# pierrepaleo/sift_pyocl

Measured on AMD Instinct MI355X. Metric: SiftPlan.keypoints throughput, 4096x4096 fp32 (Mpix/s; keypoints/s in keypoints_per_s), higher is better.
Workload: dtype f32

## Files before the change

sift_pyocl_amd/csrc/k_keypoint.hpp:

```cpp
#pragma once
#include <hip/hip_runtime.h>
#include <stdint.h>
#include "k_extrema.hpp"
#include "siftmath.hpp"

namespace siftk {

struct KpRecord { float x, y, scale, angle; uint8_t desc[128]; };
static_assert(sizeof(KpRecord) == 144, "record layout");

struct GradTaps { float xa, xb, ya, yb; bool bx, by; };

__device__ __forceinline__ GradTaps gradient_fetch(const float *__restrict__ I, int x, int y, int W, int H) {
    const size_t pos = (size_t)y * W + x;
    GradTaps t;
    t.bx = (x == 0) || (x == W - 1);
    t.by = (y == 0) || (y == H - 1);
    t.xa = I[x == W - 1 ? pos : pos + 1];
    t.xb = I[x == 0 ? pos : pos - 1];
    t.ya = I[y == 0 ? pos : pos - W];
    t.yb = I[y == H - 1 ? pos : pos + W];
    return t;
}

__device__ __forceinline__ void gradient_eval(const GradTaps &t, float &mag, float &ori) {
    float gx = t.xa - t.xb, gy = t.ya - t.yb;
// ... 8 lines not shown
    gradient_eval(gradient_fetch(I, x, y, W, H), mag, ori);
}

__device__ __forceinline__ int div_exact(int idx, int d, float inv, int &rem) {
    int q = (int)((float)idx * inv);
    rem = idx - q * d;
    if (rem < 0) { q--; rem += d; }
    else if (rem >= d) { q++; rem -= d; }
    return q;
}

#define SIFT_MAX_OCTAVES 24
#define SIFT_GROUPS 3
struct Counters {
    int n_rec;
    int tail_timeout;
    unsigned rec_word[SIFT_GROUPS];
    int g_kp[SIFT_GROUPS];
    int g_out[SIFT_GROUPS];
    int desc_next[SIFT_GROUPS];
    int n_cand[SIFT_MAX_OCTAVES + 1];
    int c_scale[SIFT_MAX_OCTAVES][3];
    int o_scale[SIFT_MAX_OCTAVES][3];
    uint32_t mm[2];
    int tail_ready[8];
};

struct OctaveTable {
    const float *base;
    long long off[SIFT_MAX_OCTAVES];
    int W[SIFT_MAX_OCTAVES], H[SIFT_MAX_OCTAVES];
    const float *gmap, *omap;
};
__device__ __forceinline__ size_t map_offset(const OctaveTable &tab, int oct, int scale) {
    return (size_t)(tab.off[oct] / 2) + (size_t)(scale - 1) * tab.W[oct] * tab.H[oct];
}

struct alignas(16) RecordSink {
    KpRecord *dev, *host;
    int dev_limit, host_limit;
};

__device__ __forceinline__ void descriptor_open(Counters *cnt, int group, int n, KpRecord *records, int rec_capacity, KpRecord *host_records,
                                                int host_capacity, RecordSink *S) {
    if (threadIdx.x == 0) {
        int base = 0;
        if (cnt) {
// ... 118 lines not shown
    if (threadIdx.x < 3 * SIFT_MAX_OCTAVES) s_hist[threadIdx.x] = 0;
    __syncthreads();
    PH_MARK(0);
    const int wave = (blockIdx.x * blockDim.x + threadIdx.x) >> 6;
    const int nwaves = (nblocks * blockDim.x) >> 6;
    const float4 *pool4 = reinterpret_cast<const float4 *>(L.pool);
    __shared__ int s_pending[4], s_base;
    int pending = 0;
    auto store_pending = [&](int slot, int count) {
        __builtin_amdgcn_wave_barrier();
        for (int e = lane; e < count; e += 64)
            if (slot + e < out_capacity) { okp[slot + e] = L.obuf[e]; oaux[slot + e] = L.oaux[e]; }
        __builtin_amdgcn_wave_barrier();
    };
    auto flush_wave = [&]() {
        int slot = 0;
        if (lane == 0) slot = atomicAdd(&cnt->g_out[group], pending);
        store_pending(__shfl(slot, 0), pending);
        pending = 0;
    };
    const bool team = count < team_below;
    const int w4 = threadIdx.x >> 6;
    const int boff = team ? 64 * w4 : 0, bstep = team ? 256 : 64;
    for (int i = first + (team ? (int)blockIdx.x : wave); i < n; i += (team ? nblocks : nwaves)) {
        const float4 k = kp[i];
        const int aux = __builtin_amdgcn_readfirstlane(kp_aux[i]);
        const int scale = aux & 0xff, oct = aux >> 8;
        const int W = tab.W[oct], H = tab.H[oct], octsize = 1 << oct;
        if (!(k.y >= 0.0f)) continue;
        const float *I = tab.base + tab.off[oct] + (size_t)scale * W * H;
        const float *Gm = MAPS ? tab.gmap + map_offset(tab, oct, scale) : nullptr;
        const float *Om = MAPS ? tab.omap + map_offset(tab, oct, scale) : nullptr;
        auto taps_at = [&](int x, int y) {
            if (!MAPS) return gradient_fetch(I, x, y, W, H);
            GradTaps t = {};
            const size_t pos = (size_t)y * W + x;
            t.xa = Gm[pos]; t.xb = Om[pos];
            return t;
        };
        const int row = (int)((double)k.y + 0.5), col = (int)((double)k.z + 0.5);
        const float sigma = ori_sigma * k.w;
        const int radius = (int)((double)sigma * 3.0);
        const int rmin = max(0, row - radius), cmin = max(0, col - radius);
        const int rmax = min(row + radius, H - 2), cmax = min(col + radius, W - 2);
        const float lim = (float)(radius * radius) + 0.5f;
        const float two_s2 = 2.0f * sigma * sigma;
        const float r_two_s2 = 1.0f / two_s2;
        const bool fast_div = two_s2 >= 1e-3f && two_s2 <= 1e6f;
        const int wc = cmax - cmin + 1, hr = rmax - rmin + 1;
// ... 439 lines not shown
```

sift_pyocl_amd/csrc/k_pyramid.hpp:

```cpp
#pragma once
#include <hip/hip_runtime.h>
#include <type_traits>
#include <stdint.h>
#include "k_xcd.hpp"

namespace siftk {

__device__ __forceinline__ uint32_t f2ord(float f) {
    uint32_t u = __float_as_uint(f);
    return (u & 0x80000000u) ? ~u : (u | 0x80000000u);
}
__device__ __forceinline__ float ord2f(uint32_t u) {
    return __uint_as_float((u & 0x80000000u) ? (u & 0x7fffffffu) : ~u);
}

__global__ void minmax_init(uint32_t *mm) { mm[0] = 0xffffffffu; mm[1] = 0u; }

__device__ __forceinline__ void minmax_reset_next(uint32_t *reset, int reset_words, int reset_ones) {
    if (reset && blockIdx.x == 0)
        for (int i = threadIdx.x; i < reset_words; i += blockDim.x) reset[i] = (i == reset_ones) ? 0xffffffffu : 0u;
}

__global__ __launch_bounds__(1024) void minmax_kernel(const float *__restrict__ img, int64_t n, uint32_t *mm, uint32_t *reset = nullptr,
                                                      int reset_words = 0, int reset_ones = -1) {
    minmax_reset_next(reset, reset_words, reset_ones);
    float lo = __builtin_inff(), hi = -__builtin_inff();
    const int64_t stride = (int64_t)gridDim.x * blockDim.x;
    int64_t i = (int64_t)blockIdx.x * blockDim.x + threadIdx.x;
    const int64_t n4 = n >> 2;
    const float4 *img4 = reinterpret_cast<const float4 *>(img);
    int64_t k = i;
    for (; k + 3 * stride < n4; k += 4 * stride) {
        const float4 v0 = img4[k], v1 = img4[k + stride], v2 = img4[k + 2 * stride], v3 = img4[k + 3 * stride];
        lo = fminf(lo, fminf(fminf(fminf(v0.x, v0.y), fminf(v0.z, v0.w)), fminf(fminf(v1.x, v1.y), fminf(v1.z, v1.w))));
        lo = fminf(lo, fminf(fminf(fminf(v2.x, v2.y), fminf(v2.z, v2.w)), fminf(fminf(v3.x, v3.y), fminf(v3.z, v3.w))));
        hi = fmaxf(hi, fmaxf(fmaxf(fmaxf(v0.x, v0.y), fmaxf(v0.z, v0.w)), fmaxf(fmaxf(v1.x, v1.y), fmaxf(v1.z, v1.w))));
        hi = fmaxf(hi, fmaxf(fmaxf(fmaxf(v2.x, v2.y), fmaxf(v2.z, v2.w)), fmaxf(fmaxf(v3.x, v3.y), fmaxf(v3.z, v3.w))));
    }
    for (; k < n4; k += stride) {
        float4 v = img4[k];
        lo = fminf(fminf(lo, v.x), fminf(v.y, fminf(v.z, v.w)));
        hi = fmaxf(fmaxf(hi, v.x), fmaxf(v.y, fmaxf(v.z, v.w)));
    }
    for (int64_t k2 = (n4 << 2) + i; k2 < n; k2 += stride) {
        float v = img[k2];
        lo = fminf(lo, v);
        hi = fmaxf(hi, v);
    }
#pragma unroll
    for (int off = 32; off > 0; off >>= 1) {
        lo = fminf(lo, __shfl_xor(lo, off));
        hi = fmaxf(hi, __shfl_xor(hi, off));
    }
    __shared__ float slo[16], shi[16];
    const int wave = threadIdx.x >> 6, nwaves = (int)blockDim.x >> 6;
    if ((threadIdx.x & 63) == 0) { slo[wave] = lo; shi[wave] = hi; }
    __syncthreads();
    if (threadIdx.x == 0) {
        lo = slo[0]; hi = shi[0];
        for (int w = 1; w < nwaves; w++) { lo = fminf(lo, slo[w]); hi = fmaxf(hi, shi[w]); }
        if (lo <= hi) {
            atomicMin(&mm[0], f2ord(lo));
            atomicMax(&mm[1], f2ord(hi));
        }
    }
}

template <int DT> __device__ __forceinline__ float load_px(const void *__restrict__ base, size_t i) {
    if constexpr (DT == 0) return static_cast<const float *>(base)[i];
    else if constexpr (DT == 1) return (float)static_cast<const uint8_t *>(base)[i];
    else if constexpr (DT == 2) return (float)static_cast<const uint16_t *>(base)[i];
    else if constexpr (DT == 3) return (float)static_cast<const uint32_t *>(base)[i];
    else if constexpr (DT == 4) return (float)static_cast<const uint64_t *>(base)[i];
    else if constexpr (DT == 5) return (float)static_cast<const int32_t *>(base)[i];
    else if constexpr (DT == 6) return (float)static_cast<const int64_t *>(base)[i];
    else {
        static_assert(DT == 8, "unsupported pixel type");
        const uint8_t *q = static_cast<const uint8_t *>(base) + 3 * i;
        const float r = (float)q[0], g = (float)q[1], b = (float)q[2];
        return (0.299f * r + 0.587f * g) + 0.114f * b;
    }
}

template <int DT> struct TypedChunk {
    static constexpr int R = (DT == 8) ? 3 : ((DT == 4 || DT == 6) ? 2 : 1);
    static constexpr int PX = (DT == 1 || DT == 8) ? 16 : (DT == 2 ? 8 : 4);
};
// ... 49 lines not shown
    for (; k < nchunks; k += stride) {
        uint4 w[C::R];
#pragma unroll
        for (int r = 0; r < C::R; r++) w[r] = img4[k * C::R + r];
        typed_chunk_minmax<DT>(w, lo, hi);
    }
    for (int64_t k2 = nchunks * C::PX + i; k2 < n; k2 += stride) {
        const float v = load_px<DT>(img, (size_t)k2);
        lo = fminf(lo, v);
        hi = fmaxf(hi, v);
    }
#pragma unroll
    for (int off = 32; off > 0; off >>= 1) {
        lo = fminf(lo, __shfl_xor(lo, off));
        hi = fmaxf(hi, __shfl_xor(hi, off));
    }
    __shared__ float slo[4], shi[4];
    const int wave = threadIdx.x >> 6;
    if ((threadIdx.x & 63) == 0) { slo[wave] = lo; shi[wave] = hi; }
    __syncthreads();
    if (threadIdx.x == 0) {
        lo = fminf(fminf(slo[0], slo[1]), fminf(slo[2], slo[3]));
        hi = fmaxf(fmaxf(shi[0], shi[1]), fmaxf(shi[2], shi[3]));
        if (lo <= hi) {
            atomicMin(&mm[0], f2ord(lo));
            atomicMax(&mm[1], f2ord(hi));
        }
    }
}

template <typename T>
__global__ void convert_kernel(const T *__restrict__ in, float *__restrict__ out, int64_t n) {
    const int64_t stride = (int64_t)gridDim.x * blockDim.x;
    for (int64_t i = (int64_t)blockIdx.x * blockDim.x + threadIdx.x; i < n; i += stride) out[i] = (float)in[i];
}
__global__ void convert_rgb_kernel(const uint8_t *__restrict__ in, float *__restrict__ out, int64_t n) {
    const int64_t stride = (int64_t)gridDim.x * blockDim.x;
    for (int64_t i = (int64_t)blockIdx.x * blockDim.x + threadIdx.x; i < n; i += stride) {
        const float r = (float)in[3 * i], g = (float)in[3 * i + 1], b = (float)in[3 * i + 2];
        out[i] = (0.299f * r + 0.587f * g) + 0.114f * b;
    }
}

template <int N> struct TapsArg { float t[N]; };

template <int N, int TX_ = 128, int TY_ = 64> struct BlurGeom {
    static constexpr int TX = TX_, TY = TY_;
    static constexpr int C = (N & 1) ? N / 2 : N / 2 - 1;
    static constexpr int ROWS = TY + N - 1;
    static constexpr int COLS = TX + N - 1;
// ... 1 lines not shown
    static constexpr int NW = (N + 3 + 3) & ~3;
    static constexpr int LDS_BYTES = ROWS * PITCH * 4;
};

__device__ __forceinline__ int reflect_index(int i, int n) {
    if (i < 0) i = -i - 1;
    else if (i > n - 1) i = 2 * n - 1 - i;
    return min(max(i, 0), n - 1);
}

template <int N, bool NORM, int DT = 0, int TX = 128, int TY = 64, int VR = 8>
__global__ __launch_bounds__(256) void blur_hv_kernel(const void *__restrict__ in, float *__restrict__ out,
                                                      int W, int H, TapsArg<N> taps,
                                                      const uint32_t *__restrict__ mm,
                                                      float *__restrict__ half) {
    using G = BlurGeom<N, TX, TY>;
    static_assert(TX % 4 == 0 && 64 % (TX / 4) == 0, "the H tasks of one row must sit in one wave");
    static_assert(TY % VR == 0, "vertical tasks tile the rows");
    extern __shared__ float4 smem4[];
    float *s = reinterpret_cast<float *>(smem4);
    const int tid = threadIdx.x;
    const int x0 = blockIdx.x * G::TX, y0 = blockIdx.y * G::TY;

    float mn = 0.f, range = 1.f;
    if (NORM) { mn = ord2f(mm[0]); range = ord2f(mm[1]) - mn; }

    for (int idx = tid; idx < G::ROWS * G::COLS; idx += 256) {
        const int row = idx / G::COLS, col = idx - row * G::COLS;
        const int gy = reflect_index(y0 - G::C + row, H);
        const int gx = reflect_index(x0 - G::C + col, W);
        float v = load_px<DT>(in, (size_t)gy * W + gx);
        if (NORM) v = 255.0f * (v - mn) / range;
        s[row * G::PITCH + col] = v;
    }
    __syncthreads();

    constexpr int HT = TX / 4;
    for (int task = tid; task < G::ROWS * HT; task += 256) {
        const int row = task / HT, t = task - row * HT;
        float *rowp = s + row * G::PITCH + 4 * t;
        float w[G::NW];
#pragma unroll
        for (int k = 0; k < G::NW / 4; k++) {
            const float4 v = *reinterpret_cast<const float4 *>(rowp + 4 * k);
            w[4 * k] = v.x; w[4 * k + 1] = v.y; w[4 * k + 2] = v.z; w[4 * k + 3] = v.w;
        }
        float a0 = 0.f, a1 = 0.f, a2 = 0.f, a3 = 0.f;
#pragma unroll
        for (int q = 0; q < N; q++) {
            const float tp = taps.t[N - 1 - q];
            a0 = a0 + w[q] * tp;
            a1 = a1 + w[q + 1] * tp;
            a2 = a2 + w[q + 2] * tp;
            a3 = a3 + w[q + 3] * tp;
        }
// ... 74 lines not shown
__global__ __launch_bounds__(64 * HW + 128) void blur_team_kernel(const void *__restrict__ in, float *__restrict__ out,
                                                          int W, int H, int nblocks, int last_subs, int rows_out,
                                                          TapsArg<N> taps, const uint32_t *__restrict__ mm,
                                                          float *__restrict__ next0,
                                                          int xcd_map, int prio) {
    constexpr int NT = 128;
    using G = March2Geom<N, NT, S>;
    using SS = SubSplit<N, S>;
    static_assert(N & 1, "marching blur needs an odd tap count");
    constexpr int BUF = G::NPS * G::PITCH * 2;
    extern __shared__ float4 smem4[];
    float *sbase = reinterpret_cast<float *>(smem4);
    const int role = __builtin_amdgcn_readfirstlane((int)threadIdx.x) >= 64 * HW ? 1 : 0;
    const int tid = role ? (int)threadIdx.x - 64 * HW : (int)threadIdx.x;
    int bx = (int)blockIdx.x, by = (int)blockIdx.y;
    if (xcd_map) {
        const int gx = (int)gridDim.x;
        const int M = xcd_contiguous(bx + gx * by, gx * (int)gridDim.y);
        by = M / gx; bx = M - by * gx;
    }
    const int x0 = bx * G::TX;
    const int ys = by * rows_out;
    const int yend = min(ys + rows_out, H);
    float mn = 0.f, range = 1.f;
    if (NORM) { mn = ord2f(mm[0]); range = ord2f(mm[1]) - mn; }

    const int gx_a = reflect_index(x0 - G::C + tid, W);
    const int gx_b = reflect_index(x0 - G::C + NT + tid, W);
    int hb_rp[G::NB], hb_col[G::NB], hb_gx[G::NB];
#pragma unroll
    for (int u = 0; u < G::NB; u++) {
        const int e = tid + NT * u;
        hb_rp[u] = (e < G::NPS * G::HALO) ? e / G::HALO : 1 << 20;
        hb_col[u] = G::TX + e % G::HALO;
        hb_gx[u] = reflect_index(x0 - G::C + hb_col[u], W);
    }
    auto ld = [&](unsigned byte_off) {
        if constexpr (DT == 0) return *reinterpret_cast<const float *>(reinterpret_cast<const char *>(in) + byte_off);
        else return load_px<DT>(in, (size_t)(byte_off >> 2));
    };
    const unsigned W4 = (unsigned)W * 4u;
    auto norm2 = [&](f32x2 v) {
        if (NORM) { v.x = 255.0f * (v.x - mn) / range; v.y = 255.0f * (v.y - mn) / range; }
        return v;
    };
    f32x2 acc[N];
#pragma unroll
    for (int k = 0; k < N; k++) acc[k] = (f32x2){0.f, 0.f};
    const int gxo = x0 + 2 * tid;
    const bool vec_store = ((W & 1) == 0) && (gxo + 1 < W);
    f32x2 pa[G::NPS], pb[G::NPS], ph[G::NB];

    auto prefetch = [&](int blk, int sub, int np) {
        const int v0 = ys - G::C + blk * N + sub * SS::RB;
        if (BLUR_ABL & 4) {
#pragma unroll
            for (int rp = 0; rp < G::NPS; rp++) { pa[rp] = (f32x2){1.f, 2.f}; pb[rp] = (f32x2){3.f, 4.f}; }
#pragma unroll
            for (int u = 0; u < G::NB; u++) ph[u] = (f32x2){5.f, 6.f};
            return;
        }
        if (v0 >= 0 && v0 + 2 * np <= H) {
            unsigned oa = ((unsigned)v0 * (unsigned)W + (unsigned)gx_a) * 4u;
            unsigned ob = ((unsigned)v0 * (unsigned)W + (unsigned)gx_b) * 4u;
#pragma unroll
            for (int rp = 0; rp < G::NPS; rp++)
                if (rp < np) {
                    pa[rp].x = ld(oa); pa[rp].y = ld(oa + W4);
                    pb[rp].x = ld(ob); pb[rp].y = ld(ob + W4);
                    oa += 2u * W4; ob += 2u * W4;
                }
        } else {
#pragma unroll
            for (int rp = 0; rp < G::NPS; rp++)
                if (rp < np) {
                    const unsigned r0 = (unsigned)reflect_index(v0 + 2 * rp, H) * W4, r1 = (unsigned)reflect_index(v0 + 2 * rp + 1, H) * W4;
                    pa[rp].x = ld(r0 + 4u * gx_a); pa[rp].y = ld(r1 + 4u * gx_a);
                    pb[rp].x = ld(r0 + 4u * gx_b); pb[rp].y = ld(r1 + 4u * gx_b);
                }
        }
#pragma unroll
        for (int u = 0; u < G::NB; u++) {
            ph[u] = (f32x2){0.f, 0.f};
            if (hb_rp[u] < np) {
                ph[u].x = ld((unsigned)reflect_index(v0 + 2 * hb_rp[u], H) * W4 + 4u * hb_gx[u]);
                ph[u].y = ld((unsigned)reflect_index(v0 + 2 * hb_rp[u] + 1, H) * W4 + 4u * hb_gx[u]);
            }
        }
    };
    auto stage = [&](float *s, int np) {
#pragma unroll
        for (int rp = 0; rp < G::NPS; rp++)
            if (rp < np) {
                *reinterpret_cast<f32x2 *>(s + (rp * G::PITCH + tid) * 2) = norm2(pa[rp]);
                *reinterpret_cast<f32x2 *>(s + (rp * G::PITCH + NT + tid) * 2) = norm2(pb[rp]);
            }
#pragma unroll
        for (int u = 0; u < G::NB; u++)
            if (hb_rp[u] < np) *reinterpret_cast<f32x2 *>(s + (hb_rp[u] * G::PITCH + hb_col[u]) * 2) = norm2(ph[u]);
    };
    auto hpass = [&](float *s, int np) {
        for (int task = tid; task < ((BLUR_ABL & 1) ? 0 : np * (NT / 2)); task += 64 * HW) {
            const int rp = task / (NT / 2), t4 = task % (NT / 2);
            float *rowp = s + (rp * G::PITCH + 4 * t4) * 2;
            f32x2 w[G::NW];
            constexpr int PRE = 4;
#pragma unroll
            for (int k = 0; k < PRE && k < G::NW / 2; k++) {
                const f32x4 v = *reinterpret_cast<const f32x4 *>(rowp + 4 * k);
                w[2 * k] = v.xy; w[2 * k + 1] = v.zw;
            }
            f32x2 a0 = {0.f, 0.f}, a1 = {0.f, 0.f}, a2 = {0.f, 0.f}, a3 = {0.f, 0.f};
#pragma unroll
            for (int q = 0; q < N; q++) {
                if ((q & 1) == 0) {
                    const int k = q / 2 + PRE;
                    if (k < G::NW / 2) {
                        const f32x4 v = *reinterpret_cast<const f32x4 *>(rowp + 4 * k);
                        w[2 * k] = v.xy; w[2 * k + 1] = v.zw;
                    }
                    __builtin_amdgcn_sched_barrier(0);
                }
// ... 137 lines not shown
template <int N, int TX, int TY> struct Tile2Geom {
    static constexpr int C = N / 2;
    static constexpr int L = 8, VR = 8;
    static constexpr int ROWS = TY + N - 1, RP = ROWS / 2;
    static constexpr int COLS = TX + N - 1;
    static constexpr int PITCH = (COLS + 1) & ~1;
    static constexpr int LDS_BYTES = RP * PITCH * 8;
};

template <int N, bool NORM, int DT = 0, int TX = 32, int TY = 64>
__global__ __launch_bounds__(256) void blur_tile2_kernel(const void *__restrict__ in, float *__restrict__ out,
                                                         int W, int H, TapsArg<N> taps,
                                                         const uint32_t *__restrict__ mm,
                                                         float *__restrict__ half) {
    using G = Tile2Geom<N, TX, TY>;
    static_assert(N & 1, "odd tap counts only");
    static_assert(TY % G::VR == 0 && TX % G::L == 0 && 64 % (TX / G::L) == 0 && G::COLS <= 128, "tile shape");
    extern __shared__ float4 smem4[];
    float *s = reinterpret_cast<float *>(smem4);
    const int tid = threadIdx.x, lane = tid & 63;
    const int wave = __builtin_amdgcn_readfirstlane(tid >> 6);
    const int x0 = blockIdx.x * TX, y0 = blockIdx.y * TY;

    float mn = 0.f, range = 1.f;
    if (NORM) { mn = ord2f(mm[0]); range = ord2f(mm[1]) - mn; }

    {
        const int c1 = lane + 64;
        const bool has0 = lane < G::COLS, has1 = c1 < G::COLS;
        const int gxa = reflect_index(x0 - G::C + lane, W), gxb = reflect_index(x0 - G::C + (has1 ? c1 : lane), W);
        const int ytop = y0 - G::C;
        const bool inside = ytop >= 0 && ytop + G::ROWS <= H;
        auto fetch = [&](int gy, int gx) {
            float v = load_px<DT>(in, (size_t)gy * W + gx);
            if (NORM) v = 255.0f * (v - mn) / range;
            return v;
        };
        f32x2 *s2 = reinterpret_cast<f32x2 *>(s);
        if (inside) {
#pragma unroll 2
            for (int rp = wave; rp < G::RP; rp += 4) {
                const int gy = ytop + 2 * rp;
                if (has0) s2[rp * G::PITCH + lane] = (f32x2){fetch(gy, gxa), fetch(gy + 1, gxa)};
                if (has1) s2[rp * G::PITCH + c1] = (f32x2){fetch(gy, gxb), fetch(gy + 1, gxb)};
            }
        } else {
#pragma unroll 2
            for (int rp = wave; rp < G::RP; rp += 4) {
                const int gy0 = reflect_index(ytop + 2 * rp, H), gy1 = reflect_index(ytop + 2 * rp + 1, H);
                if (has0) s2[rp * G::PITCH + lane] = (f32x2){fetch(gy0, gxa), fetch(gy1, gxa)};
                if (has1) s2[rp * G::PITCH + c1] = (f32x2){fetch(gy0, gxb), fetch(gy1, gxb)};
            }
        }
    }
    __syncthreads();

    constexpr int HT = TX / G::L;
    for (int task = tid; task < G::RP * HT; task += 256) {
// ... 26 lines not shown
            const int gy = y0 + r0 + j;
            if (gy < H) {
                float *o = out + (size_t)gy * W + gx;
                if (vec) *reinterpret_cast<f32x2 *>(o) = acc[j];
                else {
                    if (gx < W) o[0] = acc[j].x;
                    if (gx + 1 < W) o[1] = acc[j].y;
                }
                if (half && !(gy & 1) && (gy >> 1) < (H >> 1) && (gx >> 1) < (W >> 1))
                    half[(size_t)(gy >> 1) * (W >> 1) + (gx >> 1)] = acc[j].x;
            }
        }
    }
}


__global__ void blur_generic_pass(const float *__restrict__ in, float *__restrict__ out, int W, int H,
                                  const float *__restrict__ taps, int n, int vertical,
                                  const uint32_t *__restrict__ mm, int norm) {
    const int x = blockIdx.x * blockDim.x + threadIdx.x, y = blockIdx.y;
    if (x >= W || y >= H) return;
    const int c = (n & 1) ? n / 2 : n / 2 - 1;
    float mn = 0.f, range = 1.f;
    if (norm) { mn = ord2f(mm[0]); range = ord2f(mm[1]) - mn; }
    float acc = 0.f;
    for (int j = 0; j < n; j++) {
        float v;
        if (vertical) v = in[(size_t)reflect_index(y - c + j, H) * W + x];
        else v = in[(size_t)y * W + reflect_index(x - c + j, W)];
        if (norm) v = 255.0f * (v - mn) / range;
        acc = acc + v * taps[n - 1 - j];
    }
    out[(size_t)y * W + x] = acc;
}

__global__ __launch_bounds__(256) void shrink_kernel(const float *__restrict__ in, float *__restrict__ out, int LW, int SW, int SH) {
    const int x = (blockIdx.x * 64 + (threadIdx.x & 63)) * 4;
    const int y0 = (blockIdx.y * 4 + (threadIdx.x >> 6)) * 2;
    if (x >= SW) return;
    const bool vec_in = (LW & 1) == 0 && x + 3 < SW;
    const bool vec_out = (SW & 3) == 0;
#pragma unroll
    for (int r = 0; r < 2; r++) {
        const int y = y0 + r;
        if (y >= SH) break;
        const float *src = in + (size_t)(2 * y) * LW + 2 * x;
        float *dst = out + (size_t)y * SW + x;
        if (vec_in) {
            const float4 a = *reinterpret_cast<const float4 *>(src), b = *reinterpret_cast<const float4 *>(src + 4);
            if (vec_out) *reinterpret_cast<float4 *>(dst) = make_float4(a.x, a.z, b.x, b.z);
            else { dst[0] = a.x; dst[1] = a.z; dst[2] = b.x; dst[3] = b.z; }
        } else {
            for (int k = 0; k < 4 && x + k < SW; k++) dst[k] = src[2 * k];
        }
    }
}
inline dim3 shrink_grid(int SW, int SH) { return dim3((unsigned)((SW + 255) / 256), (unsigned)((SH + 7) / 8)); }

template <int DT = 0>
__global__ void normalize_kernel(const void *__restrict__ in, float *__restrict__ out, int64_t n,
                                 const uint32_t *__restrict__ mm) {
    const float mn = ord2f(mm[0]), range = ord2f(mm[1]) - mn;
    const int64_t stride = (int64_t)gridDim.x * blockDim.x;
    for (int64_t i = (int64_t)blockIdx.x * blockDim.x + threadIdx.x; i < n; i += stride)
        out[i] = 255.0f * (load_px<DT>(in, (size_t)i) - mn) / range;
}

}
```

sift_pyocl_amd/csrc/siftmi.hip:

```cpp
#include <hip/hip_runtime.h>
#include <hip/hip_ext.h>

#include <cmath>
#include <cstdlib>
#include <cstring>
#include <algorithm>
#include <chrono>
#include <mutex>
#include <new>
#include <string>
#include <vector>

#include "host_common.hpp"
#include "k_extrema.hpp"
#include "k_keypoint.hpp"
#include "k_descriptor.hpp"
#include "k_align.hpp"
#include "k_pyramid.hpp"
#include "k_tail.hpp"
#include "siftmath.hpp"

using namespace siftk;

static_assert(sizeof(siftmi_keypoint) == 144, "siftmi_keypoint must be 144 bytes");
// ... 356 lines not shown
    }

struct Scope {
    siftmi_plan *p; size_t idx = (size_t)-1; hipStream_t st;
    bool stop_bound = false;
    Scope(siftmi_plan *pl, const char *label, bool is_blur = false, double pixels = 0, hipStream_t s = nullptr, int octave = -1, bool record_start = true) : p(pl) {
        st = s ? s : p->stream;
        if (!p->profile || (p->profile == 1 && !(is_blur && octave == 0))) return;
        if (p->n_events == p->events.size()) {
            Event e;
            hipEventCreate(&e.a); hipEventCreate(&e.b);
            p->events.push_back(e);
        }
        idx = p->n_events++;
        Event &e = p->events[idx];
        e.label = label; e.is_blur = is_blur; e.pixels = pixels; e.octave = octave; e.launches = 1;
        if (record_start) hipEventRecord(e.a, st);
    }
    ~Scope() { if (idx != (size_t)-1 && !stop_bound) hipEventRecord(p->events[idx].b, st); }
};

double tnow() { return std::chrono::duration<double, std::micro>(std::chrono::steady_clock::now().time_since_epoch()).count(); }
float minmax_decode(uint32_t u) { uint32_t v = (u & 0x80000000u) ? (u & 0x7fffffffu) : ~u; float f; memcpy(&f, &v, 4); return f; }

int grid_for(int64_t n, int block, int max_blocks) {
    int64_t g = (n + block - 1) / block;
    if (g < 1) g = 1;
    if (g > max_blocks) g = max_blocks;
    return (int)g;
}

double contrast_threshold(const siftmi_params &par) { return 0.8 * (double)par.peak_thresh; }
float octave_edge_thresh(const siftmi_params &par, int octsize) { return (octsize <= 1) ? par.edge_thresh0 : par.edge_thresh; }


struct DetectGeom { int rows = 0, blocks = 0; };
DetectGeom detect_geometry(int W, int H, int border, int rows_opt, int min_strips, int y_lo, int y_hi) {
    DetectGeom g;
    if (!(W > 2 * border && H > 2 * border)) return g;
    g.rows = rows_opt > 0 ? rows_opt : (min_strips > 0 ? extrema_strip_rows(W, H, border, min_strips) : extrema_strip_rows(W, H, border));
    const int nx = (W - 2 * border + 61) / 62, ny = ((y_lo >= 0 ? y_hi - y_lo : H - 2 * border) + g.rows - 1) / g.rows;
    g.blocks = (nx * ny + 3) / 4;
    return g;
}

void launch_extrema(hipStream_t st, bool refine, const DetectGeom &geo, const BlurPlanes &bp, int W, int H, int border, double contrast, float edth,
// ... 351 lines not shown
    if (!rc && (prio ? hipStreamCreateWithPriority(&p->stream3, hipStreamNonBlocking, prio_hi) : hipStreamCreateWithFlags(&p->stream3, hipStreamNonBlocking)) != hipSuccess) rc = fail(SIFTMI_EDEVICE, "hipStreamCreate failed");
    if (!rc && hipEventCreateWithFlags(&p->ev_p3, SIFT_SYNC_EVENT) != hipSuccess) rc = fail(SIFTMI_EDEVICE, "hipEventCreate failed");
    p->overlap = true;
    for (int o = 0; o < p->n_oct && !rc; o++) {
        hipEvent_t e;
        if (hipEventCreateWithFlags(&e, SIFT_SYNC_EVENT) != hipSuccess) rc = fail(SIFTMI_EDEVICE, "hipEventCreate failed");
        else p->ev_pyr.push_back(e);
    }
    if (!rc) rc = p->alloc(&p->tmp, N * sizeof(float));
    if (!rc && p->n_oct > 1) rc = p->alloc(&p->tmp_later, (size_t)p->ow[1] * p->oh[1] * sizeof(float));
    if (!rc && p->n_oct > 2) rc = p->alloc(&p->tmp_below, (size_t)p->ow[2] * p->oh[2] * sizeof(float));
    if (!rc) rc = p->alloc(&p->raw, N * (dtype_size(in_dtype) > 4 ? dtype_size(in_dtype) : 4));
    if (!rc && in_dtype != SIFTMI_F32) rc = p->alloc(&p->conv, N * sizeof(float));

    if (!rc) rc = p->alloc(&p->cnt_pair, 2 * sizeof(Counters));
    if (!rc) { p->cnt = p->cnt_pair; p->mm = p->cnt->mm; }
    p->tail_cand_cap = 3 * SIFT_TAIL_MAX_PIXELS;
    if (!rc) rc = p->alloc(&p->tail_cand, (size_t)SIFT_TAIL_MAX_OCT * p->tail_cand_cap * sizeof(float4));
    if (!rc) rc = grow_lists(p, nullptr);
    if (!rc) rc = compute_schedule(p);
    if (!rc) {
        Counters zero;
        memset(&zero, 0, sizeof zero);
        zero.mm[0] = 0xffffffffu;
        if (hipMemcpy(p->cnt_pair, &zero, sizeof zero, hipMemcpyHostToDevice) != hipSuccess ||
            hipMemcpy(p->cnt_pair + 1, &zero, sizeof zero, hipMemcpyHostToDevice) != hipSuccess) rc = fail(SIFTMI_EDEVICE, "counter initialisation failed");
    }
    if (!rc) { hipEventCreate(&p->ev_first); for (hipEvent_t &e : p->ev_last) hipEventCreate(&e); }
    if (rc) { std::string keep = g_err; siftmi_plan_destroy(p); g_err = keep; return rc; }
    *out = p;
    return SIFTMI_OK;
}

int siftmi_plan_destroy(siftmi_plan *p) {
    if (!p) return SIFTMI_OK;
    hipSetDevice(p->device);
    if (p->stream) hipStreamSynchronize(p->stream);
    if (p->stream2) { hipStreamSynchronize(p->stream2); hipStreamDestroy(p->stream2); }
    if (p->stream3) { hipStreamSynchronize(p->stream3); hipStreamDestroy(p->stream3); }
    if (p->ev_p3) hipEventDestroy(p->ev_p3);
    if (p->ev_det2) hipEventDestroy(p->ev_det2);
    if (p->ev_early) hipEventDestroy(p->ev_early);
    if (p->ev_maps0) hipEventDestroy(p->ev_maps0);
    for (hipEvent_t e : p->ev_pyr) hipEventDestroy(e);
    for (void *q : p->allocs) hipFree(q);
    for (GroupLists &G : p->grp)
        for (void *q : {(void *)G.kp, (void *)G.kp_aux, (void *)G.okp, (void *)G.oaux, (void *)G.cand}) if (q) hipFree(q);
// ... 365 lines not shown
        if (!w) continue;
        if (spin) {
            hipError_t q;
            while ((q = hipStreamQuery(w)) == hipErrorNotReady) __builtin_ia32_pause();
            if (q != hipSuccess) HIPCHK(q);
        }
        HIPCHK(hipStreamSynchronize(w));
    }
    HIPCHK(hipStreamSynchronize(p->stream));
    p->in_flight = false;
    HIPCHK(hipGetLastError());
    const Counters *hcp = nullptr;
    bool tail_timed_out = false;
    for (int k = 0; k < 3; k++) {
        if (!p->wait_s[k]) continue;
        const Counters &c = p->hb->c[k];
        tail_timed_out = tail_timed_out || c.tail_timeout;
        bool complete = true;
        for (int g = 0; g < SIFT_GROUPS; g++) if (((p->groups_cur >> g) & 1u) && !(c.rec_word[g] & 0x80000000u)) complete = false;
        if (complete && (!hcp || c.n_rec >= hcp->n_rec)) hcp = &c;
    }
    if (!hcp) { drain_streams(p); return fail(SIFTMI_EDEVICE, "no complete copy of the image's counters came back"); }
    const Counters &hc = *hcp;
    p->last_min = minmax_decode(hc.mm[0]); p->last_max = minmax_decode(hc.mm[1]);
    if (!tail_timed_out && p->opt.tail_fault > 0 && p->opt.tail) { p->opt.tail_fault--; tail_timed_out = true; }
    if (tail_timed_out) {
        p->opt.tail = 0;
        p->tail_timeouts++;
        drain_streams(p);
        return fail(SIFTMI_ETAILRETRY, "octave_tail_kernel timed out waiting for the previous octave; tail launches disabled for this plan");
    }
    {
        bool grown = false;
        int rc = grow_lists(p, &hc, &grown);
        if (rc) return rc;
        if (grown) return fail(SIFTMI_EGROW, "a keypoint list was grown; the image runs again");
    }
    int64_t n = 0;
    for (int g = 0; g < SIFT_GROUPS; g++) if ((p->groups_cur >> g) & 1u) n += std::min<int64_t>(hc.g_out[g], p->grp[g].cap_out);
    n = std::min<int64_t>(std::min<int64_t>(n, hc.n_rec), p->cap_rec);
    int ovf = reference_overflow(p, hc) ? 1 : 0;
    for (int g = 0; g < SIFT_GROUPS; g++)
        if (((p->groups_cur >> g) & 1u) && (hc.g_kp[g] > p->grp[g].cap_kp || hc.g_out[g] > p->grp[g].cap_out)) ovf = 1;
    if (hc.n_rec > p->cap_rec) ovf = 1;
    for (int g = 0; g < SIFT_GROUPS; g++) {
        if (!((p->groups_cur >> g) & 1u) || p->grp[g].cap_cand <= 0) continue;
        for (int o = 0; o < p->n_oct; o++)
// ... 572 lines not shown
    Options opt = g_default_options;
    opt.xcd_map = (xcd_map & 1) ? 1 : 0;
    opt.march_prio = (xcd_map & 2) ? 0 : 2;
    opt.march_wgs = march_wgs > 0 ? march_wgs : 0;
    if ((xcd_map >> 2) & 3) opt.small_blur = ((xcd_map >> 2) & 3) - 1;
    return opt;
}

}

extern "C" {

int siftmi_stage_gaussian_taps(float sigma, int32_t size, float *out) {
    if (!out) return fail(SIFTMI_EINVAL, "null argument");
    return gaussian_taps(sigma, size, out);
}

int32_t siftmi_stage_xcd_order(int32_t id, int32_t n) { return (n > 0 && id >= 0 && id < n) ? siftk::xcd_contiguous(id, n) : -1; }

int siftmi_stage_minmax_normalize(int32_t dev, const float *in, float *out, int32_t W, int32_t H, float *mn, float *mx) {
    int rc = stage_begin(dev); if (rc) return rc;
    const size_t N = (size_t)W * H;
    DevBuf a, b, mm;
    if ((rc = a.upload(in, N * 4)) || (rc = b.alloc(N * 4)) || (rc = mm.alloc(8))) return rc;
    hipLaunchKernelGGL(minmax_init, dim3(1), dim3(1), 0, 0, mm.as<uint32_t>());
    launch_minmax(nullptr, 0, SIFTMI_F32, a.p, (int64_t)N, 256, 2048, mm.as<uint32_t>(), nullptr, 0, -1);
    launch_normalize(0, SIFTMI_F32, a.p, b.as<float>(), (int64_t)N, mm.as<uint32_t>());
    if ((rc = stage_end())) return rc;
    uint32_t h[2];
    HIPCHK(hipMemcpy(h, mm.p, 8, hipMemcpyDeviceToHost));
    if (mn) *mn = minmax_decode(h[0]);
    if (mx) *mx = minmax_decode(h[1]);
    if (out) HIPCHK(hipMemcpy(out, b.p, N * 4, hipMemcpyDeviceToHost));
    return SIFTMI_OK;
}

int siftmi_stage_blur(int32_t dev, const float *in, float *out, int32_t W, int32_t H, const float *taps, int32_t ntaps) {
    int rc = stage_begin(dev); if (rc) return rc;
    if (ntaps < 1 || ntaps > 64) return fail(SIFTMI_EINVAL, "ntaps must be in 1..64");
    const size_t N = (size_t)W * H;
    DevBuf a, b, t, dt;
    if ((rc = a.upload(in, N * 4)) || (rc = b.alloc(N * 4)) || (rc = t.alloc(N * 4))) return rc;
    Taps tp;
    if ((rc = stage_taps(taps, ntaps, dt, tp))) return rc;
    if (!launch_blur_tiled<false>(g_default_options, 0, a.as<float>(), b.as<float>(), W, H, tp, nullptr))
        launch_blur_generic(0, a.as<float>(), b.as<float>(), t.as<float>(), W, H, tp, nullptr, false);
    if ((rc = stage_end())) return rc;
    HIPCHK(hipMemcpy(out, b.p, N * 4, hipMemcpyDeviceToHost));
    return SIFTMI_OK;
}

int siftmi_stage_blur_ex(int32_t dev, const void *in, int32_t in_dtype, float *out, int32_t W, int32_t H, const float *taps, int32_t ntaps,
                         int32_t norm, int32_t xcd_map, int32_t march_wgs, int32_t *kernel_used) {
    int rc = stage_begin(dev); if (rc) return rc;
    if (!in || !out || !taps || W < 1 || H < 1) return fail(SIFTMI_EINVAL, "null argument or empty plane");
    if (ntaps < 1 || ntaps > 64) return fail(SIFTMI_EINVAL, "ntaps must be in 1..64");
    const size_t esz = dtype_size(in_dtype);
    if (!esz || in_dtype == SIFTMI_F64) return fail(SIFTMI_EINVAL, "input format %d has no fused blur", in_dtype);
    if (in_dtype != SIFTMI_F32 && !(norm && ntaps == 15)) return fail(SIFTMI_EINVAL, "typed frames enter through the normalising 15-tap blur only");
    const size_t N = (size_t)W * H;
    DevBuf a, b, t, dt, mm;
    if ((rc = a.upload(in, N * esz)) || (rc = b.alloc(N * 4)) || (rc = t.alloc(N * 4)) || (rc = mm.alloc(8))) return rc;
    Taps tp;
    if ((rc = stage_taps(taps, ntaps, dt, tp))) return rc;
    const Options opt = stage_blur_options(xcd_map, march_wgs);
    uint32_t *mmp = mm.as<uint32_t>();
    if (norm) {
        hipLaunchKernelGGL(minmax_init, dim3(1), dim3(1), 0, 0, mmp);
        launch_minmax(nullptr, 0, in_dtype, a.p, (int64_t)N, 256, in_dtype == SIFTMI_F32 ? 2048 : 256, mmp, nullptr, 0, -1);
    }
    BlurForm used = BLUR_NONE;
    if (in_dtype != SIFTMI_F32) {
        SIFTMI_TYPED_DISPATCH(in_dtype, used = launch_init_blur_dt<DT>(opt, 0, (const void *)a.p, b.as<float>(), W, H, tp, mmp));
        if (used == BLUR_NONE) return fail(SIFTMI_EINVAL, "no fused blur for input format %d", in_dtype);
    } else {
        used = norm ? launch_blur_tiled<true>(opt, 0, a.as<float>(), b.as<float>(), W, H, tp, mmp)
                    : launch_blur_tiled<false>(opt, 0, a.as<float>(), b.as<float>(), W, H, tp, mmp);
        if (used == BLUR_NONE) launch_blur_generic(0, a.as<float>(), b.as<float>(), t.as<float>(), W, H, tp, mmp, norm != 0);
    }
    if ((rc = stage_end())) return rc;
    if (kernel_used) *kernel_used = used;
    HIPCHK(hipMemcpy(out, b.p, N * 4, hipMemcpyDeviceToHost));
    return SIFTMI_OK;
}

int siftmi_stage_blur_handoff(int32_t dev, const float *in, float *out, float *half, int32_t W, int32_t H, const float *taps, int32_t ntaps,
                              int32_t xcd_map, int32_t march_wgs, int32_t *kernel_used) {
    int rc = stage_begin(dev); if (rc) return rc;
    if (!in || !out || !half || !taps || W < 1 || H < 1) return fail(SIFTMI_EINVAL, "null argument or empty plane");
    if (ntaps < 1 || ntaps > 64) return fail(SIFTMI_EINVAL, "ntaps must be in 1..64");
    const size_t N = (size_t)W * H;
// ... 305 lines not shown
```

Measured before the change: 22070.

## Spread min/max atomics over strided slots, divide by reciprocal, prefetch keypoints

The global min/max reduction now publishes into 32 slots spaced apart in memory instead of two words, which reduces atomic contention from many blocks. Consumers fold the slots back with a wave shuffle or a serial loop, and the host folds them as well. Normalisation replaces the per-pixel division with a reciprocal-based divide that falls back to true division when the operands are out of range. Separately, the descriptor loop prefetches the next keypoint record one iteration ahead. The cost is a larger counter struct and an extra fold at every consumer.

```diff
diff --git a/sift_pyocl_amd/csrc/k_keypoint.hpp b/sift_pyocl_amd/csrc/k_keypoint.hpp
--- a/sift_pyocl_amd/csrc/k_keypoint.hpp
+++ b/sift_pyocl_amd/csrc/k_keypoint.hpp
@@ -2,6 +2,7 @@
 #include <hip/hip_runtime.h>
 #include <stdint.h>
 #include "k_extrema.hpp"
+#include "k_pyramid.hpp"
 #include "siftmath.hpp"
 
 namespace siftk {
@@ -56,7 +57,7 @@
     int n_cand[SIFT_MAX_OCTAVES + 1];
     int c_scale[SIFT_MAX_OCTAVES][3];
     int o_scale[SIFT_MAX_OCTAVES][3];
-    uint32_t mm[2];
+    alignas(128) uint32_t mm[MM_WORDS];
     int tail_ready[8];
 };
 
@@ -221,9 +222,15 @@
     const bool team = count < team_below;
     const int w4 = threadIdx.x >> 6;
     const int boff = team ? 64 * w4 : 0, bstep = team ? 256 : 64;
-    for (int i = first + (team ? (int)blockIdx.x : wave); i < n; i += (team ? nblocks : nwaves)) {
-        const float4 k = kp[i];
-        const int aux = __builtin_amdgcn_readfirstlane(kp_aux[i]);
+    const int istep = team ? nblocks : nwaves;
+    int i = first + (team ? (int)blockIdx.x : wave);
+    float4 k_next = make_float4(0.f, 0.f, 0.f, 0.f);
+    int aux_next = 0;
+    if (i < n) { k_next = kp[i]; aux_next = kp_aux[i]; }
+    for (; i < n; i += istep) {
+        const float4 k = k_next;
+        const int aux = __builtin_amdgcn_readfirstlane(aux_next);
+        if (i + istep < n) { k_next = kp[i + istep]; aux_next = kp_aux[i + istep]; }
         const int scale = aux & 0xff, oct = aux >> 8;
         const int W = tab.W[oct], H = tab.H[oct], octsize = 1 << oct;
         if (!(k.y >= 0.0f)) continue;
diff --git a/sift_pyocl_amd/csrc/k_pyramid.hpp b/sift_pyocl_amd/csrc/k_pyramid.hpp
--- a/sift_pyocl_amd/csrc/k_pyramid.hpp
+++ b/sift_pyocl_amd/csrc/k_pyramid.hpp
@@ -3,6 +3,7 @@
 #include <type_traits>
 #include <stdint.h>
 #include "k_xcd.hpp"
+#include "siftmath.hpp"
 
 namespace siftk {
 
@@ -14,11 +15,62 @@
     return __uint_as_float((u & 0x80000000u) ? (u & 0x7fffffffu) : ~u);
 }
 
-__global__ void minmax_init(uint32_t *mm) { mm[0] = 0xffffffffu; mm[1] = 0u; }
+#define MM_SLOTS 32
+#define MM_STRIDE 32
+#define MM_WORDS (MM_SLOTS * MM_STRIDE)
+__global__ void minmax_init(uint32_t *mm) {
+    for (int i = threadIdx.x; i < MM_WORDS; i += blockDim.x) mm[i] = (i % MM_STRIDE == 0) ? 0xffffffffu : 0u;
+}
+__device__ __forceinline__ void minmax_publish(uint32_t *mm, float lo, float hi) {
+    if (lo <= hi) {
+        uint32_t *slot = mm + (blockIdx.x % MM_SLOTS) * MM_STRIDE;
+        atomicMin(&slot[0], f2ord(lo));
+        atomicMax(&slot[1], f2ord(hi));
+    }
+}
+__device__ __forceinline__ uint2 minmax_fold_wave(const uint32_t *__restrict__ mm) {
+    static_assert(MM_SLOTS == 32, "the fold reads one slot per lane of half a wave");
+    const uint2 w = *reinterpret_cast<const uint2 *>(mm + (threadIdx.x & (MM_SLOTS - 1)) * MM_STRIDE);
+    uint32_t lo = w.x, hi = w.y;
+#pragma unroll
+    for (int off = MM_SLOTS / 2; off > 0; off >>= 1) {
+        lo = min(lo, (uint32_t)__shfl_xor((int)lo, off));
+        hi = max(hi, (uint32_t)__shfl_xor((int)hi, off));
+    }
+    return make_uint2((uint32_t)__builtin_amdgcn_readfirstlane((int)lo), (uint32_t)__builtin_amdgcn_readfirstlane((int)hi));
+}
+__device__ __forceinline__ uint2 minmax_fold_thread(const uint32_t *__restrict__ mm) {
+    uint32_t lo = 0xffffffffu, hi = 0u;
+    for (int s = 0; s < MM_SLOTS; s++) { lo = min(lo, mm[s * MM_STRIDE]); hi = max(hi, mm[s * MM_STRIDE + 1]); }
+    return make_uint2(lo, hi);
+}
+
+#define NORM_NUM_MIN_BITS 0x26800000u
+struct NormScale { float mn, range, rb; bool fast; };
+__device__ __forceinline__ NormScale norm_scale_of(uint2 folded) {
+    NormScale n;
+    n.mn = ord2f(folded.x); n.range = ord2f(folded.y) - n.mn;
+    n.fast = n.range >= 0x1p-126f && n.range <= 0x1p64f;
+    n.rb = 1.0f / n.range;
+    return n;
+}
+__device__ __forceinline__ float norm_num(const NormScale &n, float v) { return 255.0f * (v - n.mn); }
+__device__ __forceinline__ bool norm_num_slow(float a) {
+    const uint32_t u = __float_as_uint(a);
+    return u - 1u < NORM_NUM_MIN_BITS - 1u || (u >> 31);
+}
+__device__ __forceinline__ float norm_value(const NormScale &n, float v) {
+    const float a = norm_num(n, v);
+    if (n.fast && !norm_num_slow(a)) return siftmath::div_by_reciprocal(a, n.range, n.rb);
+    return a / n.range;
+}
 
 __device__ __forceinline__ void minmax_reset_next(uint32_t *reset, int reset_words, int reset_ones) {
     if (reset && blockIdx.x == 0)
-        for (int i = threadIdx.x; i < reset_words; i += blockDim.x) reset[i] = (i == reset_ones) ? 0xffffffffu : 0u;
+        for (int i = threadIdx.x; i < reset_words; i += blockDim.x) {
+            const unsigned m = (unsigned)(i - reset_ones);
+            reset[i] = (reset_ones >= 0 && m < MM_WORDS && m % MM_STRIDE == 0) ? 0xffffffffu : 0u;
+        }
 }
 
 __global__ __launch_bounds__(1024) void minmax_kernel(const float *__restrict__ img, int64_t n, uint32_t *mm, uint32_t *reset = nullptr,
@@ -59,10 +111,7 @@
     if (threadIdx.x == 0) {
         lo = slo[0]; hi = shi[0];
         for (int w = 1; w < nwaves; w++) { lo = fminf(lo, slo[w]); hi = fmaxf(hi, shi[w]); }
-        if (lo <= hi) {
-            atomicMin(&mm[0], f2ord(lo));
-            atomicMax(&mm[1], f2ord(hi));
-        }
+        minmax_publish(mm, lo, hi);
     }
 }
 
@@ -158,10 +207,7 @@
     if (threadIdx.x == 0) {
         lo = fminf(fminf(slo[0], slo[1]), fminf(slo[2], slo[3]));
         hi = fmaxf(fmaxf(shi[0], shi[1]), fmaxf(shi[2], shi[3]));
-        if (lo <= hi) {
-            atomicMin(&mm[0], f2ord(lo));
-            atomicMax(&mm[1], f2ord(hi));
-        }
+        minmax_publish(mm, lo, hi);
     }
 }
 
@@ -209,15 +255,15 @@
     const int tid = threadIdx.x;
     const int x0 = blockIdx.x * G::TX, y0 = blockIdx.y * G::TY;
 
-    float mn = 0.f, range = 1.f;
-    if (NORM) { mn = ord2f(mm[0]); range = ord2f(mm[1]) - mn; }
+    NormScale ns = {};
+    if (NORM) ns = norm_scale_of(minmax_fold_wave(mm));
 
     for (int idx = tid; idx < G::ROWS * G::COLS; idx += 256) {
         const int row = idx / G::COLS, col = idx - row * G::COLS;
         const int gy = reflect_index(y0 - G::C + row, H);
         const int gx = reflect_index(x0 - G::C + col, W);
         float v = load_px<DT>(in, (size_t)gy * W + gx);
-        if (NORM) v = 255.0f * (v - mn) / range;
+        if (NORM) v = norm_value(ns, v);
         s[row * G::PITCH + col] = v;
     }
     __syncthreads();
@@ -338,8 +384,8 @@
     const int x0 = bx * G::TX;
     const int ys = by * rows_out;
     const int yend = min(ys + rows_out, H);
-    float mn = 0.f, range = 1.f;
-    if (NORM) { mn = ord2f(mm[0]); range = ord2f(mm[1]) - mn; }
+    NormScale ns = {};
+    if (NORM) ns = norm_scale_of(minmax_fold_wave(mm));
 
     const int gx_a = reflect_index(x0 - G::C + tid, W);
     const int gx_b = reflect_index(x0 - G::C + NT + tid, W);
@@ -356,10 +402,6 @@
         else return load_px<DT>(in, (size_t)(byte_off >> 2));
     };
     const unsigned W4 = (unsigned)W * 4u;
-    auto norm2 = [&](f32x2 v) {
-        if (NORM) { v.x = 255.0f * (v.x - mn) / range; v.y = 255.0f * (v.y - mn) / range; }
-        return v;
-    };
     f32x2 acc[N];
 #pragma unroll
     for (int k = 0; k < N; k++) acc[k] = (f32x2){0.f, 0.f};
@@ -404,16 +446,40 @@
             }
         }
     };
+    constexpr bool FASTQ = DT == 0 || DT == 1 || DT == 8;
+    auto norm_regs = [&](f32x2 &u, bool live_u, f32x2 *v, bool live_v) {
+        const float b = ns.range, rb = ns.rb;
+        u.x = norm_num(ns, u.x); u.y = norm_num(ns, u.y);
+        bool slow = live_u && (norm_num_slow(u.x) || norm_num_slow(u.y));
+        if (v) {
+            v->x = norm_num(ns, v->x); v->y = norm_num(ns, v->y);
+            slow = slow || (live_v && (norm_num_slow(v->x) || norm_num_slow(v->y)));
+        }
+        if (FASTQ && ns.fast && !__ballot(slow)) {
+            u.x = siftmath::div_by_reciprocal(u.x, b, rb); u.y = siftmath::div_by_reciprocal(u.y, b, rb);
+            if (v) { v->x = siftmath::div_by_reciprocal(v->x, b, rb); v->y = siftmath::div_by_reciprocal(v->y, b, rb); }
+        } else {
+            u.x = u.x / b; u.y = u.y / b;
+            if (v) { v->x = v->x / b; v->y = v->y / b; }
+        }
+    };
     auto stage = [&](float *s, int np) {
 #pragma unroll
         for (int rp = 0; rp < G::NPS; rp++)
             if (rp < np) {
-                *reinterpret_cast<f32x2 *>(s + (rp * G::PITCH + tid) * 2) = norm2(pa[rp]);
-                *reinterpret_cast<f32x2 *>(s + (rp * G::PITCH + NT + tid) * 2) = norm2(pb[rp]);
-            }
-#pragma unroll
-        for (int u = 0; u < G::NB; u++)
-            if (hb_rp[u] < np) *reinterpret_cast<f32x2 *>(s + (hb_rp[u] * G::PITCH + hb_col[u]) * 2) = norm2(ph[u]);
+                if (NORM) norm_regs(pa[rp], true, &pb[rp], true);
+                *reinterpret_cast<f32x2 *>(s + (rp * G::PITCH + tid) * 2) = pa[rp];
+                *reinterpret_cast<f32x2 *>(s + (rp * G::PITCH + NT + tid) * 2) = pb[rp];
+            }
+#pragma unroll
+        for (int u = 0; u < G::NB; u += 2) {
+            const bool pair = u + 1 < G::NB;
+            const int w = pair ? u + 1 : u;
+            const bool l0 = hb_rp[u] < np, l1 = pair && hb_rp[w] < np;
+            if (NORM) norm_regs(ph[u], l0, pair ? &ph[w] : nullptr, l1);
+            if (l0) *reinterpret_cast<f32x2 *>(s + (hb_rp[u] * G::PITCH + hb_col[u]) * 2) = ph[u];
+            if (l1) *reinterpret_cast<f32x2 *>(s + (hb_rp[w] * G::PITCH + hb_col[w]) * 2) = ph[w];
+        }
     };
     auto hpass = [&](float *s, int np) {
         for (int task = tid; task < ((BLUR_ABL & 1) ? 0 : np * (NT / 2)); task += 64 * HW) {
@@ -597,8 +663,8 @@
     const int wave = __builtin_amdgcn_readfirstlane(tid >> 6);
     const int x0 = blockIdx.x * TX, y0 = blockIdx.y * TY;
 
-    float mn = 0.f, range = 1.f;
-    if (NORM) { mn = ord2f(mm[0]); range = ord2f(mm[1]) - mn; }
+    NormScale ns = {};
+    if (NORM) ns = norm_scale_of(minmax_fold_wave(mm));
 
     {
         const int c1 = lane + 64;
@@ -608,7 +674,7 @@
         const bool inside = ytop >= 0 && ytop + G::ROWS <= H;
         auto fetch = [&](int gy, int gx) {
             float v = load_px<DT>(in, (size_t)gy * W + gx);
-            if (NORM) v = 255.0f * (v - mn) / range;
+            if (NORM) v = norm_value(ns, v);
             return v;
         };
         f32x2 *s2 = reinterpret_cast<f32x2 *>(s);
@@ -681,7 +747,7 @@
     if (x >= W || y >= H) return;
     const int c = (n & 1) ? n / 2 : n / 2 - 1;
     float mn = 0.f, range = 1.f;
-    if (norm) { mn = ord2f(mm[0]); range = ord2f(mm[1]) - mn; }
+    if (norm) { const uint2 f = minmax_fold_thread(mm); mn = ord2f(f.x); range = ord2f(f.y) - mn; }
     float acc = 0.f;
     for (int j = 0; j < n; j++) {
         float v;
@@ -719,7 +785,8 @@
 template <int DT = 0>
 __global__ void normalize_kernel(const void *__restrict__ in, float *__restrict__ out, int64_t n,
                                  const uint32_t *__restrict__ mm) {
-    const float mn = ord2f(mm[0]), range = ord2f(mm[1]) - mn;
+    const uint2 f = minmax_fold_thread(mm);
+    const float mn = ord2f(f.x), range = ord2f(f.y) - mn;
     const int64_t stride = (int64_t)gridDim.x * blockDim.x;
     for (int64_t i = (int64_t)blockIdx.x * blockDim.x + threadIdx.x; i < n; i += stride)
         out[i] = 255.0f * (load_px<DT>(in, (size_t)i) - mn) / range;
diff --git a/sift_pyocl_amd/csrc/siftmi.hip b/sift_pyocl_amd/csrc/siftmi.hip
--- a/sift_pyocl_amd/csrc/siftmi.hip
+++ b/sift_pyocl_amd/csrc/siftmi.hip
@@ -402,6 +402,12 @@
 
 double tnow() { return std::chrono::duration<double, std::micro>(std::chrono::steady_clock::now().time_since_epoch()).count(); }
 float minmax_decode(uint32_t u) { uint32_t v = (u & 0x80000000u) ? (u & 0x7fffffffu) : ~u; float f; memcpy(&f, &v, 4); return f; }
+void minmax_fold(const uint32_t *mm, float *mn, float *mx) {
+    uint32_t lo = 0xffffffffu, hi = 0u;
+    for (int k = 0; k < MM_SLOTS; k++) { lo = std::min(lo, mm[k * MM_STRIDE]); hi = std::max(hi, mm[k * MM_STRIDE + 1]); }
+    if (mn) *mn = minmax_decode(lo);
+    if (mx) *mx = minmax_decode(hi);
+}
 
 int grid_for(int64_t n, int block, int max_blocks) {
     int64_t g = (n + block - 1) / block;
@@ -799,7 +805,7 @@
     if (!rc) {
         Counters zero;
         memset(&zero, 0, sizeof zero);
-        zero.mm[0] = 0xffffffffu;
+        for (int k = 0; k < MM_SLOTS; k++) zero.mm[k * MM_STRIDE] = 0xffffffffu;
         if (hipMemcpy(p->cnt_pair, &zero, sizeof zero, hipMemcpyHostToDevice) != hipSuccess ||
             hipMemcpy(p->cnt_pair + 1, &zero, sizeof zero, hipMemcpyHostToDevice) != hipSuccess) rc = fail(SIFTMI_EDEVICE, "counter initialisation failed");
     }
@@ -1211,7 +1217,7 @@
     }
     if (!hcp) { drain_streams(p); return fail(SIFTMI_EDEVICE, "no complete copy of the image's counters came back"); }
     const Counters &hc = *hcp;
-    p->last_min = minmax_decode(hc.mm[0]); p->last_max = minmax_decode(hc.mm[1]);
+    minmax_fold(hc.mm, &p->last_min, &p->last_max);
     if (!tail_timed_out && p->opt.tail_fault > 0 && p->opt.tail) { p->opt.tail_fault--; tail_timed_out = true; }
     if (tail_timed_out) {
         p->opt.tail = 0;
@@ -1830,15 +1836,14 @@
     int rc = stage_begin(dev); if (rc) return rc;
     const size_t N = (size_t)W * H;
     DevBuf a, b, mm;
-    if ((rc = a.upload(in, N * 4)) || (rc = b.alloc(N * 4)) || (rc = mm.alloc(8))) return rc;
-    hipLaunchKernelGGL(minmax_init, dim3(1), dim3(1), 0, 0, mm.as<uint32_t>());
+    if ((rc = a.upload(in, N * 4)) || (rc = b.alloc(N * 4)) || (rc = mm.alloc(MM_WORDS * 4))) return rc;
+    hipLaunchKernelGGL(minmax_init, dim3(1), dim3(256), 0, 0, mm.as<uint32_t>());
     launch_minmax(nullptr, 0, SIFTMI_F32, a.p, (int64_t)N, 256, 2048, mm.as<uint32_t>(), nullptr, 0, -1);
     launch_normalize(0, SIFTMI_F32, a.p, b.as<float>(), (int64_t)N, mm.as<uint32_t>());
     if ((rc = stage_end())) return rc;
-    uint32_t h[2];
-    HIPCHK(hipMemcpy(h, mm.p, 8, hipMemcpyDeviceToHost));
-    if (mn) *mn = minmax_decode(h[0]);
-    if (mx) *mx = minmax_decode(h[1]);
+    uint32_t h[MM_WORDS];
+    HIPCHK(hipMemcpy(h, mm.p, sizeof h, hipMemcpyDeviceToHost));
+    minmax_fold(h, mn, mx);
     if (out) HIPCHK(hipMemcpy(out, b.p, N * 4, hipMemcpyDeviceToHost));
     return SIFTMI_OK;
 }
@@ -1868,13 +1873,13 @@
     if (in_dtype != SIFTMI_F32 && !(norm && ntaps == 15)) return fail(SIFTMI_EINVAL, "typed frames enter through the normalising 15-tap blur only");
     const size_t N = (size_t)W * H;
     DevBuf a, b, t, dt, mm;
-    if ((rc = a.upload(in, N * esz)) || (rc = b.alloc(N * 4)) || (rc = t.alloc(N * 4)) || (rc = mm.alloc(8))) return rc;
+    if ((rc = a.upload(in, N * esz)) || (rc = b.alloc(N * 4)) || (rc = t.alloc(N * 4)) || (rc = mm.alloc(MM_WORDS * 4))) return rc;
     Taps tp;
     if ((rc = stage_taps(taps, ntaps, dt, tp))) return rc;
     const Options opt = stage_blur_options(xcd_map, march_wgs);
     uint32_t *mmp = mm.as<uint32_t>();
     if (norm) {
-        hipLaunchKernelGGL(minmax_init, dim3(1), dim3(1), 0, 0, mmp);
+        hipLaunchKernelGGL(minmax_init, dim3(1), dim3(256), 0, 0, mmp);
         launch_minmax(nullptr, 0, in_dtype, a.p, (int64_t)N, 256, in_dtype == SIFTMI_F32 ? 2048 : 256, mmp, nullptr, 0, -1);
     }
     BlurForm used = BLUR_NONE;
```

Result: no change. 22010 (median of 2 runs) (-0.3%).
